# tool-recommender-bot/logparser

Hardware: AMD Instinct MI355X
Metric: GB/s (and lines/s) of 'combined' log parsed per GPU and per 8xMI355X node (higher is better)
Workload: dtype u8

## Files before the change

logparser_amd/csrc/kernels_common.h:

```cpp
#pragma once
#include <hip/hip_runtime.h>

#ifndef LP_KERNEL_TU
#define LP_KERNEL_TU 1
#endif

#include <algorithm>

#include "kernels.h"
#include "lp_device.h"
#include "lp_owner.h"

namespace lp {
namespace {

constexpr int CHUNK = 64 * 1024;
constexpr int NL_THREADS = 256;
constexpr int PW = 64;

typedef uint32_t u32x4 __attribute__((ext_vector_type(4)));

__device__ __forceinline__ uint32_t byte_eq(uint32_t w, uint32_t c4) {
    uint32_t x = w ^ c4;
    return ~(((x & 0x7F7F7F7Fu) + 0x7F7F7F7Fu) | x | 0x7F7F7F7Fu);
}
__device__ __forceinline__ uint32_t bits16(uint32_t m0, uint32_t m1, uint32_t m2, uint32_t m3) {
    return bcls::nib(m0) | (bcls::nib(m1) << 4) | (bcls::nib(m2) << 8) | (bcls::nib(m3) << 12);
}

__device__ __forceinline__ uint32_t term_bits(uint4 v, const uint8_t* p, uint64_t pos, uint64_t nbytes) {
    uint32_t lf = bits16(byte_eq(v.x, 0x0A0A0A0Au), byte_eq(v.y, 0x0A0A0A0Au), byte_eq(v.z, 0x0A0A0A0Au),
                         byte_eq(v.w, 0x0A0A0A0Au));
    uint32_t cr = bits16(byte_eq(v.x, 0x0D0D0D0Du), byte_eq(v.y, 0x0D0D0D0Du), byte_eq(v.z, 0x0D0D0D0Du),
                         byte_eq(v.w, 0x0D0D0D0Du));
    if (pos + 16 > nbytes) {
        const uint32_t live = nbytes > pos ? (1u << (uint32_t)(nbytes - pos)) - 1u : 0u;
        lf &= live;
        cr &= live;
    }
    if (cr) {
        uint32_t next_lf = lf >> 1;
        if ((cr & 0x8000u) && pos + 16 < nbytes && p[pos + 16] == '\n') next_lf |= 0x8000u;
        cr &= ~next_lf;
    }
    return lf | cr;
}
__device__ __forceinline__ uint32_t term16(const uint8_t* p, uint64_t pos, uint64_t nbytes) {
    uint4 v = make_uint4(0, 0, 0, 0);
    if (pos + 16 <= nbytes && ((uintptr_t)(p + pos) & 15) == 0) {
        v = *reinterpret_cast<const uint4*>(p + pos);
    } else {
        uint32_t w[4] = {0, 0, 0, 0};
        for (uint64_t k = pos; k < pos + 16 && k < nbytes; ++k) w[(k - pos) >> 2] |= (uint32_t)p[k] << (8 * ((k - pos) & 3));
        v = make_uint4(w[0], w[1], w[2], w[3]);
    }
    return term_bits(v, p, pos, nbytes);
}

__device__ __forceinline__ int lane_id() {
    return (int)__builtin_amdgcn_mbcnt_hi(~0u, __builtin_amdgcn_mbcnt_lo(~0u, 0u));
}

struct WaveStack {
    uint32_t* base;
    __device__ uint32_t& operator[](int k) const { return base[k * PW]; }
};

template <typename LN>
__device__ __forceinline__ LN owner_line(const LN& L, int own) {
    LN R = L;
    R.o = (uint32_t)__shfl((int)L.o, own);
    R.n = __shfl(L.n, own);
    if constexpr (!LN::has_masks)
        R.b = reinterpret_cast<decltype(L.b)>(__shfl((unsigned long long)(uintptr_t)L.b, own));
    return R;
}

struct WaveLines {
    int64_t li0, li, lend;
    bool active;
    uint64_t s, e, w0, w1;
    int n;
};
__device__ __forceinline__ WaveLines wave_lines(const Columns& C, int64_t wave, int64_t n_lines, uint64_t nbytes) {
    WaveLines W;
    W.li0 = wave * PW;
    W.li = W.li0 + (int64_t)lane_id();
    W.active = W.li < n_lines;
    W.lend = W.li0 + PW < n_lines ? W.li0 + PW : n_lines;
    W.s = W.e = 0;
    if (W.active) {
        W.s = C.line_off[W.li];
        W.e = C.line_off[W.li + 1] - 1;
    }
    W.n = (int)((W.e - W.s) > (uint64_t)0x7FFFFFFF ? 0x7FFFFFFF : (W.e - W.s));
    W.w0 = C.line_off[W.li0] & ~15ull;
    W.w1 = C.line_off[W.lend];
    if (W.w1 > nbytes) W.w1 = nbytes;
    return W;
}

__device__ __forceinline__ int crlf_len(int n, uint32_t last) { return n - (n > 0 && last == '\r' ? 1 : 0); }
__device__ __forceinline__ int crlf_len_hbm(const uint8_t* buf, const WaveLines& W) {
    return W.active ? crlf_len(W.n, W.n > 0 ? buf[W.e - 1] : 0u) : W.n;
}

__device__ __forceinline__ bool stage_window(const uint8_t* __restrict__ buf, uint64_t nbytes, uint64_t w0, uint64_t w1,
                                             uint8_t* win, uint16_t* msk16) {
    const int lane = lane_id();
    const int nv = (int)((w1 - w0 + 15) >> 4);
    const int nv4 = (nv + 3) & ~3;
    uint32_t bad = 0;
    constexpr int SB = 20;
    const uint64_t full_end = nbytes & ~15ull;
    for (int k0 = lane; k0 < nv4; k0 += SB * PW) {
        u32x4 v[SB];
#pragma unroll
        for (int j = 0; j < SB; ++j) {
            const int k = k0 + j * PW;
            const uint64_t p = w0 + 16ull * k;
            v[j] = u32x4{0, 0, 0, 0};
            if (k < nv && p + 16 <= full_end) v[j] = __builtin_nontemporal_load(reinterpret_cast<const u32x4*>(buf + p));
        }
#pragma unroll
        for (int j = 0; j < SB; ++j) {
            const int k = k0 + j * PW;
            if (k >= nv4) continue;
            const uint64_t p = w0 + 16ull * k;
            if (k < nv && p + 16 > full_end) {
                auto word = [&](uint64_t q) {
                    uint32_t w = 0;
#pragma unroll
                    for (int b = 0; b < 4; ++b) w |= q + b < nbytes ? (uint32_t)buf[q + b] << (8 * b) : 0u;
                    return w;
                };
                v[j] = u32x4{word(p), word(p + 4), word(p + 8), word(p + 12)};
            }
            *reinterpret_cast<u32x4*>(win + 16 * k) = v[j];
            uint32_t m0, m1, g = 0, lf, other, cr;
            bcls::classify16p(v[j][0], v[j][1], v[j][2], v[j][3], m0, m1, g, lf, other);
            if (other) bcls::classify16c(v[j][0], v[j][1], v[j][2], v[j][3], g, cr);
            if (k < nv) bad |= g;
            msk16[8 * (k >> 2) + (k & 3)] = (uint16_t)m0;
            msk16[8 * (k >> 2) + 4 + (k & 3)] = (uint16_t)m1;
        }
    }
    return !__any(bad != 0);
}

struct WaveCounts {
    uint32_t act = 0, ok = 0, bad = 0, written = 0;
    uint32_t gathered = 0;
    __device__ __forceinline__ void store(LP_G uint32_t* wave_counts, int64_t wave) const {
        if (lane_id() == 0) {
            uint4 c, d;
            c.x = act;
            c.y = ok;
            c.z = bad;
            c.w = act - ok - bad;
            d.x = written;
            d.y = gathered;
            d.z = d.w = 0;
            uint4* wc = reinterpret_cast<uint4*>(wave_counts + WC_WORDS * (size_t)wave);
            wc[0] = c;
            wc[1] = d;
        }
    }
    __device__ __forceinline__ void store(const Columns& C, int64_t wave) const { store(C.wave_counts, wave); }
};

template <bool MULTI, typename LN>
__device__ __forceinline__ void parse_wave(const Program& P, const Elem* elems, const Columns& C, const LN& L,
                                           bool active, int64_t li, WaveStack stk, bool clean, WaveCounts& WC) {
    LineOut o;
    o.status = ST_OK;
    LP_PROF(1);
    if (active) phase1<MULTI>(P, elems, L, o, stk, C, li, clean, P.n_fmt > 1 ? (int)C.fmt_id[li] : 0);
    LP_PROF(9);
    if (active) write_line(P, o, C, li);
    if (active && !P.has_phase2()) C.arena_base[li] = 0;
    WC.act += (uint32_t)__popcll(__ballot(active));
    WC.ok += (uint32_t)__popcll(__ballot(active && o.status == ST_OK));
    WC.bad += (uint32_t)__popcll(__ballot(active && o.status == ST_BAD));
}

__device__ __forceinline__ u32x4 load16(const uint8_t* __restrict__ buf, uint64_t nbytes, uint64_t p) {
    if (p + 16 <= nbytes) return *reinterpret_cast<const u32x4*>(buf + p);
    uint32_t w[4] = {0, 0, 0, 0};
    for (int c = 0; c < 16; ++c) w[c >> 2] |= p + c < nbytes ? (uint32_t)buf[p + c] << (8 * (c & 3)) : 0u;
    return u32x4{w[0], w[1], w[2], w[3]};
}

__device__ __forceinline__ void load_elems(const Program& P, Elem* s_elems) {
    for (int k = lane_id(); k < P.n_elems; k += PW) s_elems[k] = P.elems[k];
}

__device__ __forceinline__ int lsb64(uint64_t m) { return (int)__builtin_ctzll(m); }
__device__ __forceinline__ int msb64(uint64_t m) { return 63 - (int)__builtin_clzll(m); }

template <typename T>
__device__ __forceinline__ T wave_incl_scan(T x) {
    const int lane = lane_id();
    for (int d = 1; d < 64; d <<= 1) {
        const T y = __shfl_up(x, d);
        if (lane >= d) x += y;
    }
    return x;
}
__device__ __forceinline__ uint32_t wave_incl_scan_dpp(uint32_t x) {
    constexpr int ROW_SHR = 0x110, ROW_BCAST15 = 0x142, ROW_BCAST31 = 0x143;
    x += (uint32_t)__builtin_amdgcn_update_dpp(0, (int)x, ROW_SHR + 1, 0xF, 0xF, false);
    x += (uint32_t)__builtin_amdgcn_update_dpp(0, (int)x, ROW_SHR + 2, 0xF, 0xF, false);
    x += (uint32_t)__builtin_amdgcn_update_dpp(0, (int)x, ROW_SHR + 4, 0xF, 0xF, false);
    x += (uint32_t)__builtin_amdgcn_update_dpp(0, (int)x, ROW_SHR + 8, 0xF, 0xF, false);
    x += (uint32_t)__builtin_amdgcn_update_dpp(0, (int)x, ROW_BCAST15, 0xA, 0xF, false);
    x += (uint32_t)__builtin_amdgcn_update_dpp(0, (int)x, ROW_BCAST31, 0xC, 0xF, false);
    return x;
}
__device__ __forceinline__ uint32_t lane_value(uint32_t x, int l) {
    return (uint32_t)__builtin_amdgcn_readlane((int)x, l);
}
template <typename T>
__device__ __forceinline__ T wave_sum(T x) {
    for (int d = 32; d > 0; d >>= 1) x += __shfl_xor(x, d);
    return x;
}

}
}
```

logparser_amd/csrc/lp_device.h:

```cpp
#pragma once
#include <cstddef>
#include <type_traits>
#include <utility>

#include "lp_program.h"
#include "lp_fixed.h"

namespace lp {

enum : int { ST_OK = 0, ST_BAD = 1, ST_FALLBACK = 2,
             ST_REDO = 3,
             ST_REPAIR = 4 };

#if defined(LP_PROFILE) && defined(__HIP__)
static __device__ unsigned long long g_prof[PROF_WAVES * PROF_POINTS];
#endif
#if defined(LP_PROFILE) && defined(__HIP_DEVICE_COMPILE__)
__device__ __forceinline__ void lp_prof_mark(int k) {
    const unsigned long long t = clock64();
    const unsigned w = blockIdx.x - PROF_W0;
    const uint64_t act = __ballot(1);
    if (w < (unsigned)PROF_WAVES && (int)threadIdx.x % 64 == (int)__builtin_ctzll(act))
        __builtin_nontemporal_store(t, &g_prof[w * PROF_POINTS + k]);
}
__device__ __forceinline__ void lp_prof_acc(int k, unsigned long long& t0) {
    const unsigned long long t = clock64();
    const unsigned w = blockIdx.x - PROF_W0;
    const uint64_t act = __ballot(1);
    if (w < (unsigned)PROF_WAVES && (int)threadIdx.x % 64 == (int)__builtin_ctzll(act))
        g_prof[w * PROF_POINTS + k] += t - t0;
    t0 = t;
}
#define LP_PROF(k) lp_prof_mark(k)
#define LP_PT_DECL unsigned long long lp_pt = clock64();
#define LP_PACC(k) lp_prof_acc(k, lp_pt)
#else
#define LP_PROF(k)
#define LP_PT_DECL
#define LP_PACC(k)
#endif
#if defined(LP_PROFILE) && defined(__HIP_DEVICE_COMPILE__)
#define LP_PROF_EL_BEGIN() unsigned long long lp_el_t = clock64();
#define LP_PROF_EL_END(i) if ((i) < 32) lp_prof_acc(64 + (i), lp_el_t);
#else
#define LP_PROF_EL_BEGIN()
#define LP_PROF_EL_END(i)
#endif

__host__ __device__ LP_INLINE bool is_ws(uint32_t c) { return c == ' ' || (c >= 9 && c <= 13); }
__host__ __device__ LP_INLINE bool is_digit(uint32_t c) { return c - '0' < 10u; }
__host__ __device__ LP_INLINE bool is_hex(uint32_t c) { return is_digit(c) || ((c | 32u) - 'a') < 6u; }
__host__ __device__ LP_INLINE bool is_alpha(uint32_t c) { return ((c | 32u) - 'a') < 26u; }
__host__ __device__ LP_INLINE bool is_alnum(uint32_t c) { return is_alpha(c) || is_digit(c); }
__host__ __device__ LP_INLINE uint32_t hexv(uint32_t c) { return c <= '9' ? c - '0' : (c | 32u) - 'a' + 10; }
__host__ __device__ LP_INLINE int utf8_len(uint32_t c) { return c < 0x80 ? 1 : c < 0xE0 ? 2 : c < 0xF0 ? 3 : 4; }
__host__ __device__ LP_INLINE bool uri_needs_encode(uint32_t c) {
    constexpr uint64_t LO = 0x5000000500000000ull | 0x1FFFFFFFFull;
    constexpr uint64_t HI = 0xB800000178000000ull;
    return c >= 0x80 || (((c < 64 ? LO : HI) >> (c & 63)) & 1u);
}

__host__ __device__ LP_INLINE uint32_t load_word(const uint8_t* p) {
#if defined(__HIP_DEVICE_COMPILE__)
    return *reinterpret_cast<const uint32_t*>(__builtin_assume_aligned(p, 4));
#else
    uint32_t v;
    __builtin_memcpy(&v, p, 4);
    return v;
#endif
}
#if defined(__HIP__)
typedef const __attribute__((address_space(3))) uint8_t* lds_bytes;
typedef const __attribute__((address_space(3))) uint32_t* lds_words;
__device__ LP_INLINE uint32_t load_word(lds_bytes p) { return *(lds_words)p; }
#endif
#if defined(__HIP_DEVICE_COMPILE__) && defined(LP_KERNEL_TU)
__device__ LP_INLINE uint32_t load_word(const LP_G uint8_t* p) {
    return *reinterpret_cast<const LP_G uint32_t*>(__builtin_assume_aligned(p, 4));
}
#endif

enum : int {
    MC_QUOTE = 0,
    MC_UEV = 1,
    MC_WS = 2,
    MC_N = 2
};
__host__ __device__ LP_INLINE uint64_t mask_load(const uint64_t* p) { return *p; }
#if defined(__HIP__)
typedef const __attribute__((address_space(3))) uint64_t* lds_u64;
__device__ LP_INLINE uint64_t mask_load(lds_u64 p) { return *p; }
#endif
struct NoMasks {};
static_assert((int)MC_QUOTE == fs::ACLS_QUOTE, "lp_fixed.h names the QUOTE class by its value");

template <typename Ptr, typename MPtr = NoMasks, int NPL = 2>
struct LineT {
    Ptr b;
    uint32_t o;
    int n;
    MPtr m = MPtr{};
    static constexpr bool has_masks = !std::is_same<MPtr, NoMasks>::value;
    static constexpr bool in_arena = false;
    __host__ __device__ LP_INLINE uint32_t operator[](int i) const { return b[o + i]; }
    __host__ __device__ LP_INLINE uint32_t word(uint32_t w) const { return load_word(b + 4 * w); }
    __host__ __device__ LP_INLINE uint32_t word_or0(uint32_t w) const {
        return 4 * w < o + (uint32_t)n ? load_word(b + 4 * w) : 0u;
    }
    __host__ __device__ LP_INLINE uint64_t mask(int c, uint32_t w) const {
        if constexpr (NPL == 1) {
            return mask_load(m + w);
        } else {
            return mask_load(m + 2 * w + (c == MC_QUOTE ? 0 : 1));
        }
    }
};
using Line = LineT<const uint8_t*>;
using MLine = LineT<const uint8_t*, const uint64_t*>;
using ULine = LineT<const uint8_t*, const uint64_t*, 1>;

template <typename Ptr>
struct ArenaLineT : LineT<Ptr> {
    uint32_t rb;
    static constexpr bool in_arena = true;
};

template <typename LN>
__host__ __device__ LP_INLINE uint64_t src_ref(const LN& L, int x, int n) {
    if constexpr (LN::in_arena) return mkref(L.rb + (uint32_t)x, (uint32_t)n, true);
    else return mkref((uint32_t)x, (uint32_t)n, false);
}

namespace swar {
constexpr uint32_t ONES = 0x01010101u, HI = 0x80808080u, LO7 = 0x7F7F7F7Fu;
__host__ __device__ LP_INLINE uint32_t eq(uint32_t w, uint32_t c) {
    const uint32_t x = w ^ (c * ONES);
    return ~(((x & LO7) + LO7) | x | LO7);
}
__host__ __device__ LP_INLINE uint32_t ge(uint32_t w, uint32_t n) { return (((w & LO7) + (0x80u - n) * ONES) | w) & HI; }
__host__ __device__ LP_INLINE uint32_t lt(uint32_t w, uint32_t n) { return ~ge(w, n) & HI; }
__host__ __device__ LP_INLINE uint32_t ws(uint32_t w) { return eq(w, ' ') | (ge(w, 9) & lt(w, 14)); }
__host__ __device__ LP_INLINE uint32_t digit(uint32_t w) { return ge(w, '0') & lt(w, '9' + 1); }
__host__ __device__ LP_INLINE uint32_t hex(uint32_t w) {
    const uint32_t l = w | 0x20202020u;
    return digit(w) | (ge(l, 'a') & lt(l, 'g') & ~(w & HI));
}
__host__ __device__ LP_INLINE uint32_t upper(uint32_t w) { return ge(w, 'A') & lt(w, 'Z' + 1); }
__host__ __device__ LP_INLINE uint32_t guard_bad(uint32_t w) { return (lt(w, 0x20) & ~eq(w, '\t')) | ge(w, 0x7F); }
__host__ __device__ LP_INLINE uint32_t guard_ctl(uint32_t w) { return (lt(w, 0x20) & ~eq(w, '\t')) | eq(w, 0x7F); }
__host__ __device__ LP_INLINE uint32_t needs_encode(uint32_t w) {
    return lt(w, 0x21) | ge(w, 0x7F) | (ge(w, '{') & lt(w, '~')) | (ge(w, '[') & lt(w, '_')) | eq(w, '`') |
           eq(w, '<') | eq(w, '>') | eq(w, '"');
}
__host__ __device__ LP_INLINE int first(uint32_t m) {
#if defined(__HIP_DEVICE_COMPILE__)
    return (int)(__builtin_ctz(m) >> 3);
#else
    return (int)(__builtin_ctz(m) >> 3);
#endif
}
__host__ __device__ LP_INLINE int last(uint32_t m) { return (int)((31 - __builtin_clz(m)) >> 3); }
__host__ __device__ LP_INLINE int count(uint32_t m) { return __builtin_popcount(m); }
}


namespace bcls {
constexpr uint32_t LO0 = 0x08040081u, LO1 = 0x00080800u;
constexpr uint32_t LO2 = 0x38020200u, LO3 = 0x10502230u;
constexpr uint32_t HI0 = 0x100D0002u, HI1 = 0x20806000u;
__host__ __device__ LP_INLINE uint32_t perm(uint32_t s0, uint32_t s1, uint32_t sel) {
#if defined(__HIP_DEVICE_COMPILE__)
    return __builtin_amdgcn_perm(s0, s1, sel);
#else
    const uint64_t v = ((uint64_t)s0 << 32) | s1;
    uint32_t r = 0;
    for (int i = 0; i < 4; ++i) r |= (uint32_t)((v >> (8 * ((sel >> (8 * i)) & 7))) & 0xFFu) << (8 * i);
    return r;
#endif
}
__host__ __device__ LP_INLINE uint32_t bits(uint32_t w) {
    const uint32_t s = w & 0x07070707u;
    const uint32_t p1 = perm(LO1, LO0, s), p2 = perm(LO3, LO2, s);
    const uint32_t m8 = ((w >> 3) & 0x01010101u) * 0xFFu;
    const uint32_t rl = (p2 & m8) | (p1 & ~m8);
    const uint32_t hb = ((w >> 7) & 0x01010101u) * 0xFFu;
    return (rl & perm(HI1, HI0, (w >> 4) & 0x07070707u) & ~hb) | (hb & 0x08080808u);
}
constexpr uint32_t NA_LO0 = 0x0303010Bu, NA_LO1 = 0x01030301u, NA_LO2 = 0x11010101u, NA_LO3 = 0x47251115u;
constexpr uint32_t NA_HI0 = 0x04020101u, NA_HI1 = 0x50083008u;
__host__ __device__ LP_INLINE uint32_t nonauth_bits(uint32_t w) {
    const uint32_t s = w & 0x07070707u;
    const uint32_t p1 = perm(NA_LO1, NA_LO0, s), p2 = perm(NA_LO3, NA_LO2, s);
    const uint32_t m8 = ((w >> 3) & 0x01010101u) * 0xFFu;
    return ((p2 & m8) | (p1 & ~m8)) & perm(NA_HI1, NA_HI0, (w >> 4) & 0x07070707u);
}
__host__ __device__ LP_INLINE uint32_t nib(uint32_t hb) { return (((hb >> 7) * 0x204081u) >> 21) & 15u; }
__host__ __device__ LP_INLINE uint32_t uev_hb(uint32_t r) { return (((r & swar::LO7) + swar::LO7) | r) & swar::HI; }
__host__ __device__ LP_INLINE uint32_t pack16(uint32_t h0, uint32_t h1, uint32_t h2, uint32_t h3);
__host__ __device__ LP_INLINE uint32_t classify16u(uint32_t w0, uint32_t w1, uint32_t w2, uint32_t w3) {
    return pack16(uev_hb(bits(w0)), uev_hb(bits(w1)), uev_hb(bits(w2)), uev_hb(bits(w3)));
}
__host__ __device__ LP_INLINE uint32_t pack16(uint32_t h0, uint32_t h1, uint32_t h2, uint32_t h3) {
#if defined(__HIP_DEVICE_COMPILE__)
    const uint32_t lo = __builtin_amdgcn_udot4(h1, 0x80402010u, __builtin_amdgcn_udot4(h0, 0x08040201u, 0u, false), false);
    const uint32_t hi = __builtin_amdgcn_udot4(h3, 0x80402010u, __builtin_amdgcn_udot4(h2, 0x08040201u, 0u, false), false);
    return (lo >> 7) | (hi << 1);
#else
    return nib(h0) | (nib(h1) << 4) | (nib(h2) << 8) | (nib(h3) << 12);
#endif
}
__host__ __device__ LP_INLINE void classify16p(uint32_t w0, uint32_t w1, uint32_t w2, uint32_t w3, uint32_t& p0,
                                               uint32_t& p1, uint32_t& bad, uint32_t& lf, uint32_t& other) {
    const uint32_t w[4] = {w0, w1, w2, w3};
    uint32_t q[4], le[4], l[4], o = 0, hi = 0;
    LP_UNROLL for (int k = 0; k < 4; ++k) {
        const uint32_t lo7 = w[k] & swar::LO7;
        le[k] = ~((lo7 + 0x5F5F5F5Fu) | w[k]) & swar::HI;
        const uint32_t lt = ~((lo7 + 0x60606060u) | w[k]) & swar::HI;
        hi |= ((lo7 + 0x01010101u) | w[k]) & swar::HI;
        q[k] = swar::eq(w[k], '"');
        l[k] = swar::eq(w[k], '\n');
        o |= lt & ~l[k];
    }
    p0 = pack16(q[0], q[1], q[2], q[3]);
    p1 = pack16(le[0], le[1], le[2], le[3]);
    lf = pack16(l[0], l[1], l[2], l[3]);
    bad |= hi;
    other = o;
}
__host__ __device__ LP_INLINE void classify16c(uint32_t w0, uint32_t w1, uint32_t w2, uint32_t w3, uint32_t& bad,
                                               uint32_t& cr) {
    const uint32_t w[4] = {w0, w1, w2, w3};
    uint32_t c[4];
    LP_UNROLL for (int k = 0; k < 4; ++k) {
        const uint32_t lt = ~(((w[k] & swar::LO7) + 0x60606060u) | w[k]) & swar::HI;
        c[k] = swar::eq(w[k], '\r');
        bad |= lt & ~(c[k] | swar::eq(w[k], '\n') | swar::eq(w[k], '\t'));
    }
    cr = pack16(c[0], c[1], c[2], c[3]);
}
__host__ __device__ LP_INLINE int class_of(uint32_t c) { return c == '"' ? (int)MC_QUOTE : -1; }
}

inline void build_masks(const uint8_t* buf, uint32_t n, uint64_t* masks) {
    for (uint32_t i = 0; i < MC_N * (n / 64); ++i) masks[i] = 0;
    for (uint32_t k = 0; 16 * k < n; ++k) {
        uint32_t w[4];
        for (int j = 0; j < 4; ++j) __builtin_memcpy(&w[j], buf + 16 * k + 4 * j, 4);
        uint32_t a, b, bad = 0, lf, other;
        bcls::classify16p(w[0], w[1], w[2], w[3], a, b, bad, lf, other);
        const int sh = 16 * (k & 3);
        masks[2 * (k >> 2)] |= (uint64_t)a << sh;
        masks[2 * (k >> 2) + 1] |= (uint64_t)b << sh;
    }
}

inline void build_uev_plane(const uint8_t* buf, uint32_t n, uint64_t* plane) {
    for (uint32_t i = 0; i < n / 64; ++i) plane[i] = 0;
    for (uint32_t k = 0; 16 * k < n; ++k) {
        uint32_t w[4];
        for (int j = 0; j < 4; ++j) __builtin_memcpy(&w[j], buf + 16 * k + 4 * j, 4);
        plane[k >> 2] |= (uint64_t)bcls::classify16u(w[0], w[1], w[2], w[3]) << (16 * (k & 3));
    }
}

__host__ __device__ LP_INLINE int ctz64(uint64_t m) { return __builtin_ctzll(m); }
__host__ __device__ LP_INLINE int msb64(uint64_t m) { return 63 - __builtin_clzll(m); }
__host__ __device__ LP_INLINE int popc64(uint64_t m) { return __builtin_popcountll(m); }

template <typename LN, typename F>
__host__ __device__ LP_INLINE int find_fwd(const LN& L, int from, int to, F cls) {
    if (from >= to) return to;
    const uint32_t A = L.o + (uint32_t)from, E = L.o + (uint32_t)to;
    uint32_t W = A >> 2;
    uint32_t m = cls(L.word(W)) & (swar::HI << (8 * (A & 3)));
    for (;;) {
        if (m) {
            const uint32_t p = (W << 2) + (uint32_t)swar::first(m);
            return p < E ? (int)(p - L.o) : to;
        }
        ++W;
        if ((W << 2) >= E) return to;
        m = cls(L.word(W));
    }
}
template <typename LN, typename F>
__host__ __device__ LP_INLINE int find_bwd(const LN& L, int hi, int lo, F cls) {
    if (hi < lo) return -1;
    const uint32_t A = L.o + (uint32_t)hi, S = L.o + (uint32_t)lo;
    uint32_t W = A >> 2;
    uint32_t m = cls(L.word(W)) & (swar::HI >> (8 * (3 - (A & 3))));
    for (;;) {
        if (m) {
            const uint32_t p = (W << 2) + (uint32_t)swar::last(m);
            return p >= S ? (int)(p - L.o) : -1;
        }
        if ((W << 2) <= S) return -1;
        --W;
        m = cls(L.word(W));
    }
}
template <typename LN, typename F>
__host__ __device__ LP_INLINE uint32_t count_in(const LN& L, int a, int b, F cls) {
    if (a >= b) return 0;
    const uint32_t A = L.o + (uint32_t)a, E = L.o + (uint32_t)b;
    const uint32_t W0 = A >> 2, W1 = (E - 1) >> 2;
    uint32_t c = 0;
    for (uint32_t W = W0; W <= W1; ++W) {
        uint32_t m = cls(L.word(W));
        if (W == W0) m &= swar::HI << (8 * (A & 3));
        if (W == W1) m &= swar::HI >> (8 * (3 - ((E - 1) & 3)));
        c += (uint32_t)swar::count(m);
    }
    return c;
}

template <typename LN>
__host__ __device__ LP_INLINE int mfind_fwd(const LN& L, int c, int from, int to) {
    if (from >= to) return to;
    const uint32_t A = L.o + (uint32_t)from, E = L.o + (uint32_t)to;
    uint32_t W = A >> 6;
    uint64_t m = L.mask(c, W) & (~0ull << (A & 63));
    for (;;) {
        if (m) {
            const uint32_t p = (W << 6) + (uint32_t)ctz64(m);
            return p < E ? (int)(p - L.o) : to;
        }
        ++W;
        if ((W << 6) >= E) return to;
        m = L.mask(c, W);
    }
}
template <typename LN>
__host__ __device__ LP_INLINE int mfind_bwd(const LN& L, int c, int hi, int lo) {
    if (hi < lo) return -1;
    const uint32_t A = L.o + (uint32_t)hi, S = L.o + (uint32_t)lo;
    uint32_t W = A >> 6;
    uint64_t m = L.mask(c, W) & (~0ull >> (63 - (A & 63)));
    for (;;) {
        if (m) {
            const uint32_t p = (W << 6) + (uint32_t)msb64(m);
            return p >= S ? (int)(p - L.o) : -1;
        }
        if ((W << 6) <= S) return -1;
        --W;
        m = L.mask(c, W);
    }
}

template <typename LN, typename F>
__host__ __device__ LP_INLINE bool for_uev(const LN& L, int a, int b, F&& f) {
    if (a >= b) return true;
    const uint32_t A = L.o + (uint32_t)a, E = L.o + (uint32_t)b;
    if constexpr (LN::has_masks) {
        const uint32_t W1 = (E - 1) >> 6;
        const uint64_t last = ~0ull >> (63 - ((E - 1) & 63));
        uint32_t W = A >> 6;
        uint64_t m = L.mask(MC_UEV, W) & (~0ull << (A & 63));
        if (W == W1) m &= last;
        auto next = [&](int& q) {
            while (!m) {
                if (++W > W1) return false;
                m = L.mask(MC_UEV, W);
                if (W == W1) m &= last;
            }
            q = (int)((W << 6) + (uint32_t)ctz64(m) - L.o);
            m &= m - 1;
            return true;
        };
        int q;
        if (!next(q)) return true;
        uint32_t c = L[q];
        for (;;) {
            int q2 = 0;
            const bool more = next(q2);
            const uint32_t c2 = more ? L[q2] : 0u;
            if (!f(q, c)) return false;
            if (!more) return true;
            q = q2;
            c = c2;
        }
    } else {
        const uint32_t W0 = A >> 2, W1 = (E - 1) >> 2;
        for (uint32_t W = W0; W <= W1; ++W) {
            const uint32_t w = L.word(W);
            uint32_t m = bcls::uev_hb(bcls::bits(w));
            if (W == W0) m &= swar::HI << (8 * (A & 3));
            if (W == W1) m &= swar::HI >> (8 * (3 - ((E - 1) & 3)));
            while (m) {
                const int k = swar::first(m);
                m &= m - 1;
                if (!f((int)((W << 2) + (uint32_t)k - L.o), (w >> (8 * k)) & 0xFFu)) return false;
            }
        }
    }
    return true;
}

template <typename LN, typename F>
__host__ __device__ LP_INLINE bool for_uev_w(const LN& L, int a, int b, F&& f) {
    if (a >= b) return true;
    const uint32_t A = L.o + (uint32_t)a, E = L.o + (uint32_t)b;
    if constexpr (LN::has_masks) {
        const uint32_t W1 = (E - 1) >> 6;
        const uint64_t last = ~0ull >> (63 - ((E - 1) & 63));
        uint32_t W = A >> 6;
        uint64_t m = L.mask(MC_UEV, W) & (~0ull << (A & 63));
        if (W == W1) m &= last;
        auto next = [&](int& q) {
            while (!m) {
                if (++W > W1) return false;
                m = L.mask(MC_UEV, W);
                if (W == W1) m &= last;
            }
            q = (int)((W << 6) + (uint32_t)ctz64(m) - L.o);
            m &= m - 1;
            return true;
        };
        int q;
        if (!next(q)) return true;
        uint32_t w = load_u32_at(L, q);
        for (;;) {
            int q2 = 0;
            const bool more = next(q2);
            const uint32_t w2 = more ? load_u32_at(L, q2) : 0u;
            if (!f(q, w)) return false;
            if (!more) return true;
            q = q2;
            w = w2;
        }
    } else {
        return for_uev(L, a, b, [&](int q, uint32_t) { return f(q, load_u32_at(L, q)); });
    }
}

template <typename LN>
__host__ __device__ LP_INLINE uint32_t count_uev(const LN& L, int a, int b) {
    if (a >= b) return 0;
    const uint32_t A = L.o + (uint32_t)a, E = L.o + (uint32_t)b;
    uint32_t c = 0;
    if constexpr (LN::has_masks) {
        const uint32_t W0 = A >> 6, W1 = (E - 1) >> 6;
        for (uint32_t W = W0; W <= W1; ++W) {
            uint64_t m = L.mask(MC_UEV, W);
            if (W == W0) m &= ~0ull << (A & 63);
            if (W == W1) m &= ~0ull >> (63 - ((E - 1) & 63));
            c += (uint32_t)popc64(m);
        }
    } else {
        const uint32_t W0 = A >> 2, W1 = (E - 1) >> 2;
        for (uint32_t W = W0; W <= W1; ++W) {
            uint32_t m = bcls::uev_hb(bcls::bits(L.word(W)));
            if (W == W0) m &= swar::HI << (8 * (A & 3));
            if (W == W1) m &= swar::HI >> (8 * (3 - ((E - 1) & 3)));
            c += (uint32_t)swar::count(m);
        }
    }
    return c;
}

template <typename LN>
__host__ __device__ LP_INLINE int find_ws(const LN& L, int from, int to) {
    if constexpr (LN::has_masks) return mfind_fwd(L, MC_WS, from, to);
    else return find_fwd(L, from, to, [](uint32_t w) { return swar::ws(w); });
}

template <typename LN>
__host__ __device__ LP_INLINE uint32_t load_u32_at(const LN& L, int p) {
    const uint32_t A = L.o + (uint32_t)p;
    const uint32_t w0 = L.word(A >> 2), w1 = L.word_or0((A >> 2) + 1);
#if defined(__HIP_DEVICE_COMPILE__)
    return __builtin_amdgcn_alignbyte(w1, w0, A & 3);
#else
    return (uint32_t)((((uint64_t)w1 << 32) | w0) >> (8 * (A & 3)));
#endif
}

struct Bytes28 {
    uint32_t v[7];
    __host__ __device__ LP_INLINE uint32_t operator[](int k) const { return (v[k >> 2] >> (8 * (k & 3))) & 0xFFu; }
};
template <typename LN>
__host__ __device__ LP_INLINE Bytes28 load28(const LN& L, int p) {
    const uint32_t A = L.o + (uint32_t)p, W = A >> 2, s = A & 3;
    uint32_t w[8];
    LP_UNROLL for (int j = 0; j < 7; ++j) w[j] = L.word(W + j);
    w[7] = L.word_or0(W + 7);
    Bytes28 r;
    LP_UNROLL for (int j = 0; j < 7; ++j) {
#if defined(__HIP_DEVICE_COMPILE__)
        r.v[j] = __builtin_amdgcn_alignbyte(w[j + 1], w[j], s);
#else
        r.v[j] = (uint32_t)((((uint64_t)w[j + 1] << 32) | w[j]) >> (8 * s));
#endif
    }
    return r;
}

template <int N>
struct RegArr {
    static constexpr int size = N;
#if defined(__HIP_DEVICE_COMPILE__)
    typedef uint32_t vec_t __attribute__((ext_vector_type(N)));
    vec_t v;
#else
    uint32_t v[N];
#endif
    template <size_t... J>
    __host__ __device__ LP_INLINE uint32_t get_(int k, std::index_sequence<J...>) const {
        uint32_t r = 0;
        ((r = ((int)J == k) ? v[J] : r), ...);
        return r;
    }
    template <size_t... J>
    __host__ __device__ LP_INLINE void set_(int k, uint32_t x, std::index_sequence<J...>) {
        ((v[J] = ((int)J == k) ? x : v[J]), ...);
    }
    template <typename F, size_t... J>
    __host__ __device__ LP_INLINE void each_(F&& f, std::index_sequence<J...>) const {
        (f((int)J, v[J]), ...);
    }
    __host__ __device__ LP_INLINE uint32_t get(int k) const { return get_(k, std::make_index_sequence<N>{}); }
    __host__ __device__ LP_INLINE uint32_t get_u(int k) const { return v[k]; }
    __host__ __device__ LP_INLINE void set_u(int k, uint32_t x) {
        if ((unsigned)k < (unsigned)N) v[k] = x;
    }
    __host__ __device__ LP_INLINE void set(int k, uint32_t x) { set_(k, x, std::make_index_sequence<N>{}); }
    __host__ __device__ LP_INLINE void fill(uint32_t x) { set_all(x, std::make_index_sequence<N>{}); }
    template <size_t... J>
    __host__ __device__ LP_INLINE void set_all(uint32_t x, std::index_sequence<J...>) { ((v[J] = x), ...); }
    template <typename F>
    __host__ __device__ LP_INLINE void each(F&& f) const { each_(f, std::make_index_sequence<N>{}); }
};

template <typename LN>
__host__ __device__ LP_INLINE bool lit_at(const Program& P, const LN& L, int pos, const ElemV& e) {
    const int len = e.lit_len;
    if (pos + len > L.n) return false;
    if (len <= 4) {
        const uint32_t keep = len == 4 ? 0xFFFFFFFFu : ((1u << (8 * len)) - 1u);
        return ((load_u32_at(L, pos) ^ e.lit4) & keep) == 0;
    }
// ... 3157 lines not shown
```

logparser_amd/csrc/parse_chunk.h:

```cpp
#pragma once
#include "kernels_common.h"

namespace lp {

namespace {


constexpr int MAXS = PW + 1;
#ifndef LP_CHUNK_MAXW
#define LP_CHUNK_MAXW 10
#endif
#ifndef LP_CHUNK_LMAX
#define LP_CHUNK_LMAX 54
#endif
#ifndef LP_MF_WPE
#define LP_MF_WPE 3
#endif
#ifndef LP_CHUNK_LMAX_MF
#define LP_CHUNK_LMAX_MF 58
#endif
constexpr uint64_t CS_AGG = 1ull << 62, CS_INC = 1ull << 63, CS_CNT = CS_AGG - 1;

__device__ __forceinline__ LP_G uint64_t* line_off_w(const Columns& C) { return const_cast<LP_G uint64_t*>(C.line_off); }

constexpr uint64_t CHK_OVF_LINE = 1, CHK_EXCESS = 2, CHK_QUEUE = 3;
__device__ __forceinline__ void check_fail(const Columns& C, uint64_t kind, uint64_t a, uint64_t b, uint64_t c,
                                           uint64_t d) {
    if (atomicAdd(&C.meta->err, 1ull) == 0) {
        C.meta->err_info[0] = kind;
        C.meta->err_info[1] = a;
        C.meta->err_info[2] = b;
        C.meta->err_info[3] = c;
        C.meta->err_info[4] = d;
    }
}

__device__ __forceinline__ void queue_line(const Columns& C, uint64_t li) {
    const uint64_t q = atomicAdd(&C.meta->ovf_lines, 1ull);
    if (q <= (uint64_t)C.cap_lines) C.ovf_lines[q] = (uint32_t)li;
    else check_fail(C, CHK_QUEUE, 0, q, li, (uint64_t)C.cap_lines + 1);
}

__device__ __forceinline__ uint32_t below(uint64_t b) {
    return __builtin_amdgcn_mbcnt_hi((uint32_t)(b >> 32), __builtin_amdgcn_mbcnt_lo((uint32_t)b, 0u));
}

struct ChunkScan {
    uint32_t count;
    uint64_t end_term;
    bool clean;
};

__device__ __forceinline__ ChunkScan stage_chunk(const uint8_t* __restrict__ buf, uint64_t nbytes, uint64_t w0,
                                                 uint64_t w1, uint64_t t_lo, uint64_t t_hi, uint32_t first,
                                                 uint8_t* win, uint16_t* msk16, uint32_t* starts) {
    const int lane = lane_id();
    const int nv = (int)((w1 - w0 + 15) >> 4);
    const int nv4 = (nv + 3) & ~3;
    if ((nv & (PW - 1)) == 0 && w0 + 16ull * nv <= (nbytes & ~15ull)) {
        for (int k0 = 0; k0 < nv; k0 += PW)
            __builtin_amdgcn_global_load_lds((const __attribute__((address_space(1))) void*)(buf + w0 + 16ull * (k0 + lane)),
                                             (__attribute__((address_space(3))) void*)(win + 16 * k0), 16, 0, 0);
        asm volatile("s_waitcnt vmcnt(0)" ::: "memory");
    } else {
        for (int k = lane; k < nv4; k += PW) {
            u32x4 v = u32x4{0, 0, 0, 0};
            if (k < nv) v = load16(buf, nbytes, w0 + 16ull * k);
            *reinterpret_cast<u32x4*>(win + 16 * k) = v;
        }
    }
    const uint32_t nrel = nbytes - w0 < 16ull * (uint64_t)(nv4 + 1) ? (uint32_t)(nbytes - w0) : 16u * (uint32_t)(nv4 + 1);
    const uint32_t tl = (uint32_t)(t_lo - w0), th = (uint32_t)(t_hi - w0);
    uint32_t bad = 0;
    uint32_t run = first;
    uint32_t end_rel = ~0u;
    u32x4 vn = lane < nv4 ? *reinterpret_cast<const u32x4*>(win + 16 * lane) : u32x4{0, 0, 0, 0};
    for (int k0 = 0; k0 < nv4; k0 += PW) {
        const int k = k0 + lane;
        const uint32_t q = 16u * (uint32_t)k;
        const uint32_t r0 = 16u * (uint32_t)k0, r1 = r0 + 16u * PW;
        const bool inner = r0 >= tl && r1 <= th && r1 <= nrel && k0 + PW <= nv;
        uint32_t tm = 0;
        const u32x4 v = vn;
        if (k + PW < nv4) vn = *reinterpret_cast<const u32x4*>(win + 16 * (k + PW));
        if (k < nv4) {
            uint32_t m0, m1, g = 0, lf, other;
            bcls::classify16p(v[0], v[1], v[2], v[3], m0, m1, g, lf, other);
            msk16[8 * (k >> 2) + (k & 3)] = (uint16_t)m0;
            msk16[8 * (k >> 2) + 4 + (k & 3)] = (uint16_t)m1;
            tm = lf;
            if (other) {
                uint32_t cr;
                bcls::classify16c(v[0], v[1], v[2], v[3], g, cr);
                if (cr) {
                    const uint64_t p = w0 + q;
                    uint32_t next_lf = lf >> 1;
                    if ((cr & 0x8000u) && p + 16 < nbytes && buf[p + 16] == '\n') next_lf |= 0x8000u;
                    tm |= cr & ~next_lf;
                }
            }
            if (inner) {
                bad |= g;
            } else {
                if (k < nv) bad |= g;
                if (q + 16 > nrel) tm &= nrel > q ? (1u << (nrel - q)) - 1u : 0u;
            }
        }
        uint32_t ms = tm;
        if (!inner) {
            uint32_t me = 0;
            if (q < tl) ms &= tl - q >= 16 ? 0u : ~0u << (tl - q);
            if (q + 16 > th) {
                const uint32_t lo = th > q ? (1u << (th - q)) - 1u : 0u;
                me = tm & ~lo;
                ms &= lo;
            }
            if (me) end_rel = min(end_rel, q + (uint32_t)__builtin_ctz(me));
        }
        const uint32_t c = (uint32_t)__popc(ms);
        const uint64_t b0 = __ballot(c & 1u), b1 = __ballot(c & 2u);
        uint32_t excl = below(b0) + 2 * below(b1);
        uint32_t tot = (uint32_t)(__popcll(b0) + 2 * __popcll(b1));
        const uint64_t bh = __ballot(c >= 4u);
        if (bh) {
            const uint64_t b2 = __ballot(c & 4u), b3 = __ballot(c & 8u), b4 = __ballot(c & 16u);
            excl += 4 * below(b2) + 8 * below(b3) + 16 * below(b4);
            tot += (uint32_t)(4 * __popcll(b2) + 8 * __popcll(b3) + 16 * __popcll(b4));
        }
        uint32_t r = run + excl;
        run += tot;
        for (uint32_t m = ms; m; m &= m - 1, ++r)
            if (r < (uint32_t)MAXS) starts[r] = q + (uint32_t)__builtin_ctz(m) + 1u;
    }
    ChunkScan S;
    S.count = run;
    for (int d = 32; d > 0; d >>= 1) end_rel = min(end_rel, (uint32_t)__shfl_xor((int)end_rel, d));
    S.end_term = end_rel == ~0u ? ~0ull : w0 + end_rel;
    S.clean = !__any(bad != 0);
    return S;
}

__device__ __forceinline__ void chunk_publish(LP_G uint64_t* st, int64_t c, uint64_t count) {
    if (lane_id() == 0) __hip_atomic_store(&st[c], CS_AGG | count, __ATOMIC_RELAXED, __HIP_MEMORY_SCOPE_AGENT);
}

__device__ __noinline__ void chunk_scanner(LP_G uint64_t* st, int64_t n_chunks) {
    constexpr int PER = 8;
    const int lane = lane_id();
    uint64_t run = 0;
    int64_t c = 0;
    while (c < n_chunks) {
        uint64_t v[PER];
#pragma unroll
        for (int i = 0; i < PER; ++i) {
            const int64_t idx = c + PER * lane + i;
            v[i] = idx < n_chunks ? __hip_atomic_load(&st[idx], __ATOMIC_RELAXED, __HIP_MEMORY_SCOPE_AGENT) : 0ull;
        }
        int pub = 0;
        uint64_t sum = 0;
        bool stop = false;
#pragma unroll
        for (int i = 0; i < PER; ++i) {
            stop = stop || !(v[i] & CS_AGG);
            if (!stop) { sum += v[i] & CS_CNT; ++pub; }
        }
        const uint64_t full = __ballot(pub == PER);
        const int L = full == ~0ull ? PW : (int)__builtin_ctzll(~full);
        const uint64_t mine = lane <= L ? sum : 0ull;
        const uint64_t incl = wave_incl_scan(mine);
        const uint64_t total = __shfl(incl, PW - 1);
        const int pub_L = L < PW ? __shfl(pub, L) : 0;
        if (lane <= L) {
            uint64_t r = run + incl - mine;
#pragma unroll
            for (int i = 0; i < PER; ++i) {
                if (i >= pub) break;
                r += v[i] & CS_CNT;
                __hip_atomic_store(&st[c + PER * lane + i], CS_INC | r, __ATOMIC_RELAXED, __HIP_MEMORY_SCOPE_AGENT);
            }
        }
        const int64_t adv = (int64_t)L * PER + pub_L;
        run += total;
        c += adv;
        if (adv == 0) __builtin_amdgcn_s_sleep(8);
    }
}

constexpr uint32_t CHUNK_WAIT_MAX = 1u << 14;
__device__ __forceinline__ uint64_t chunk_base(LP_G uint64_t* st, int64_t c, uint64_t count, int wait_max) {
    if (wait_max < 0 && (wait_max != -2 || (c & 1))) return ~0ull;
    uint64_t v = 0;
    const uint32_t lim = wait_max <= 0 ? CHUNK_WAIT_MAX : (uint32_t)wait_max;
    if (lane_id() == 0) {
        for (uint32_t it = 0;; ++it) {
            v = __hip_atomic_load(&st[c], __ATOMIC_RELAXED, __HIP_MEMORY_SCOPE_AGENT);
            if (v & CS_INC) break;
            if (it >= lim) { v = ~0ull; break; }
            __builtin_amdgcn_s_sleep(4);
        }
    }
    v = __shfl(v, 0);
    return v == ~0ull ? ~0ull : (v & CS_CNT) - count;
}

__device__ __noinline__ void chunk_excess(const uint8_t* __restrict__ buf, uint64_t nbytes, const Columns& C,
                                         const uint8_t* win, uint64_t w0, uint64_t w1, uint64_t t_lo, uint64_t t_hi,
                                         uint32_t first, uint64_t base, int64_t chunk, uint32_t count) {
    const int lane = lane_id();
    const int nv = (int)((w1 - w0 + 15) >> 4);
    uint32_t run = first;
    for (int k0 = 0; k0 < nv; k0 += PW) {
        const int k = k0 + lane;
        const uint64_t p = w0 + 16ull * k;
        uint32_t ms = 0;
        if (k < nv) {
            const u32x4 v = *reinterpret_cast<const u32x4*>(win + 16 * k);
            ms = term_bits(make_uint4(v[0], v[1], v[2], v[3]), buf, p, nbytes);
            if (p < t_lo) ms &= t_lo - p >= 16 ? 0u : ~0u << (uint32_t)(t_lo - p);
            if (p + 16 > t_hi) ms &= t_hi > p ? (1u << (uint32_t)(t_hi - p)) - 1u : 0u;
        }
        const uint32_t c = (uint32_t)__popc(ms);
        const uint32_t incl = wave_incl_scan(c);
        uint32_t r = run + incl - c;
        run += (uint32_t)__shfl((int)incl, 63);
        for (uint32_t m = ms; m; m &= m - 1, ++r) {
            if (r < (uint32_t)PW) continue;
            const uint64_t li = base + r;
            if ((int64_t)li >= C.cap_lines) continue;
            line_off_w(C)[li] = p + (uint64_t)__builtin_ctz(m) + 1;
            queue_line(C, li);
        }
    }
    if (lane == 0 && run != count) {
        check_fail(C, CHK_EXCESS, (uint64_t)chunk, run, count, base);
        if (C.meta->err_info[1] == (uint64_t)chunk) {
            C.meta->err_info[5] = w0;
            C.meta->err_info[6] = w1;
            C.meta->err_info[7] = t_lo;
            C.meta->err_info[8] = t_hi;
            C.meta->err_info[9] = first;
            C.meta->err_info[10] = (uint64_t)(uintptr_t)win;
            C.meta->err_info[11] = nbytes;
            C.meta->err_info[12] = (uint64_t)(uintptr_t)buf;
        }
    }
}

template <bool LA, bool SIMPLE, bool MF = false, int SHAPE = FS_NONE>
__device__ __forceinline__ void parse_chunk(const uint8_t* __restrict__ buf, uint64_t nbytes, const Program& P,
                                            const Columns& C, const Elem* s_elems, uint8_t* smem, int64_t c,
                                            int64_t n_chunks, uint32_t cb, uint32_t win_cap, uint32_t stk_words,
                                            int direct, int wait_max, bool second) {
    const uint64_t c0 = (uint64_t)c * cb;
    const uint64_t c1 = c0 + cb < nbytes ? c0 + cb : nbytes;
    const int lane = lane_id();
    WaveStack stk{reinterpret_cast<uint32_t*>(smem + 16 * P.n_elems) + lane};
    uint32_t* starts = reinterpret_cast<uint32_t*>(smem + 16 * P.n_elems + 4 * stk_words);
    uint8_t* win = smem + 16 * P.n_elems + 4 * stk_words + 16 * ((4 * MAXS + 15) / 16);
    uint16_t* msk16 = reinterpret_cast<uint16_t*>(win + win_cap);
    const uint64_t w0 = c0 >= 64 ? c0 - 64 : 0;
    const uint64_t w1 = w0 + win_cap < nbytes ? w0 + win_cap : nbytes;
    const uint64_t t_lo = c0 ? c0 - 1 : 0, t_hi = c1 - 1;
    const uint32_t first = c0 == 0 ? 1u : 0u;
    if (first && lane == 0) starts[0] = 0;
    LP_PROF(0);
    const ChunkScan S = stage_chunk(buf, nbytes, w0, w1, t_lo, t_hi, first, win, msk16, starts);
    if (!second) chunk_publish(C.chunk_state, c, S.count);
    LP_PROF(60);
    __syncthreads();
    const uint32_t nl = S.count < (uint32_t)PW ? S.count : (uint32_t)PW;
    const bool has = (uint32_t)lane < nl;
    uint32_t s = 0, e = 0;
    bool known = false;
    if (has) {
        s = starts[lane];
        if ((uint32_t)lane + 1 < S.count) {
            e = starts[lane + 1] - 1;
            known = true;
        } else if (S.end_term != ~0ull) {
            e = (uint32_t)(S.end_term - w0);
            known = true;
        } else if (w1 == nbytes) {
            e = (uint32_t)(nbytes - w0);
            known = true;
        }
    }
    const bool lds_line = has && known && !direct;
    const int n = lds_line ? crlf_len((int)(e - s), e > s ? win[e - 1] : 0u) : 0;
    const LineT<lds_bytes, lds_u64> L{(lds_bytes)win, lds_line ? s : 0u, n, (lds_u64)reinterpret_cast<uint64_t*>(msk16)};
    LineOut o;
    o.status = ST_OK;
    o.tdone = o.smdone = o.bipdone = 0;
    LP_PROF(1);
    uint32_t mword = 0;
    if constexpr (MF) {
        if (lds_line) {
            bool redo = false;
            mword = fmt_match_word<false>(P, s_elems, L, stk, S.clean, &redo, &o.caps);
            const uint32_t mm = mword & 0xFFu;
            if (redo || (mword >> 8) || (mm & (mm - 1))) o.status = ST_REDO;
            else if (mm == 0) o.status = ST_BAD;
            else phase1<true, LA, false, false, true>(P, s_elems, L, o, stk, C, 0, S.clean, __builtin_ctz(mm));
        }
    } else {
#if defined(LP_DFS_IN_CHUNKS)
        if (lds_line) phase1<false, LA, SIMPLE, true>(P, s_elems, L, o, stk, C, 0, S.clean, 0);
#else
        if (lds_line) phase1<false, LA, SIMPLE, false, false, SHAPE>(P, s_elems, L, o, stk, C, 0, S.clean, 0);
#endif
    }
    LP_PROF(9);
    const uint64_t base = chunk_base(C.chunk_state, c, S.count, second ? (int)CHUNK_WAIT_MAX : wait_max);
    if (base == ~0ull) {
        if (lane == 0) {
            const uint64_t q = atomicAdd(&C.meta->deferred, 1ull);
            if (q < (uint64_t)n_chunks) C.deferred_chunks[q] = (uint32_t)c;
            else check_fail(C, CHK_QUEUE, 1, q, (uint64_t)c, (uint64_t)n_chunks);
        }
        return;
    }
    LP_PROF(61);
    const int64_t cap = C.cap_lines;
    const int64_t li = (int64_t)base + lane;
    const bool mine = has && li < cap;
    if (mine) line_off_w(C)[li] = w0 + s;
    if constexpr (MF) {
        if (mine) C.fmt_match[li] = (uint16_t)mword;
    }
    const bool redo = lds_line && o.status == ST_REDO;
    const bool row = mine && lds_line && !redo;
    if (mine && (!lds_line || redo)) queue_line(C, (uint64_t)li);
    {
        const uint32_t nredo = (uint32_t)__popcll(__ballot(mine && redo));
        if (nredo && lane == 0) atomicAdd(&C.meta->dfs_lines, (unsigned long long)nredo);
    }
    if (row) {
        write_line(P, o, C, li);
        if (!P.has_phase2()) C.arena_base[li] = 0;
    }
    if (S.count > (uint32_t)PW)
        chunk_excess(buf, nbytes, C, win, w0, w1, t_lo, t_hi, first, base, c, S.count);
    if (c == n_chunks - 1 && lane == 0) {
        const uint64_t total = base + S.count;
        C.meta->n_lines = total;
        C.meta->cap_ovf = (int64_t)total > cap ? 1ull : 0ull;
        if ((int64_t)total <= cap) {
            const uint8_t last = buf[nbytes - 1];
            line_off_w(C)[total] = last == '\n' || last == '\r' ? nbytes : nbytes + 1;
        }
    }
    WaveCounts WC;
    WC.act = (uint32_t)__popcll(__ballot(row));
    WC.ok = (uint32_t)__popcll(__ballot(row && o.status == ST_OK));
    WC.bad = (uint32_t)__popcll(__ballot(row && o.status == ST_BAD));
    WC.store(C.chunk_counts, c);
    LP_PROF(62);
}

template <bool LA, bool SIMPLE, bool MF, int SHAPE = FS_NONE>
__global__ __launch_bounds__(PW, MF ? LP_MF_WPE : 2) void k_parse_chunks(const uint8_t* __restrict__ buf, uint64_t nbytes,
                                                     const DeviceArgs* __restrict__ args, uint32_t cb, uint32_t win_cap,
                                                     uint32_t stk_words, int direct, int wait_max) {
    const Program& P = args->prog;
    const Columns& C = args->cols;
    const int64_t n_chunks = (int64_t)((nbytes + cb - 1) / cb);
    if (blockIdx.x == 0) {
        chunk_scanner(C.chunk_state, n_chunks);
        return;
    }
    const int64_t c = (int64_t)blockIdx.x - 1;
    if ((uint64_t)c * cb >= nbytes) return;
    extern __shared__ __attribute__((aligned(16))) uint8_t smem[];
    Elem* s_elems = reinterpret_cast<Elem*>(smem);
    load_elems(P, s_elems);
    parse_chunk<LA, SIMPLE, MF, SHAPE>(buf, nbytes, P, C, s_elems, smem, c, n_chunks, cb, win_cap, stk_words, direct,
                                       wait_max, false);
}

template <bool LA, bool SIMPLE, bool MF>
__global__ __launch_bounds__(PW, 2) void k_parse_deferred(const uint8_t* __restrict__ buf, uint64_t nbytes,
                                                       const DeviceArgs* __restrict__ args, uint32_t cb,
                                                       uint32_t win_cap, uint32_t stk_words, int direct) {
    const Program& P = args->prog;
    const Columns& C = args->cols;
    const uint64_t nd = C.meta->deferred;
    if (blockIdx.x >= nd) return;
    const int64_t n_chunks = (int64_t)((nbytes + cb - 1) / cb);
    extern __shared__ __attribute__((aligned(16))) uint8_t smem[];
    Elem* s_elems = reinterpret_cast<Elem*>(smem);
    load_elems(P, s_elems);
    for (uint64_t q = blockIdx.x; q < nd; q += gridDim.x) {
        parse_chunk<LA, SIMPLE, MF>(buf, nbytes, P, C, s_elems, smem, (int64_t)C.deferred_chunks[q], n_chunks, cb,
                                    win_cap, stk_words, direct, 0, true);
        __syncthreads();
    }
}

}
}
```

Baseline: 702.9.

## Classify 64-byte blocks per lane in chunk scan instead of 16-byte vectors

The chunk scan loop now has each lane classify a 64-byte block (four 16-byte vectors) and build 64-bit terminator masks. A wave therefore covers 4KB per iteration, which cuts loop trips and the ballot-based prefix counting per byte by about four times, and the mask writes become single 16-byte stores. In exchange each lane holds more registers, uses more ballot rounds when per-lane counts are high, and the tail handling now works at 64-byte granularity. A profiling marker is also added after the LDS load wait.

Result: faster. 745.0, median of 6 (+6.0%).

```diff
diff --git a/logparser_amd/csrc/kernels_common.h b/logparser_amd/csrc/kernels_common.h
--- a/logparser_amd/csrc/kernels_common.h
+++ b/logparser_amd/csrc/kernels_common.h
@@ -19,6 +19,7 @@
 constexpr int PW = 64;
 
 typedef uint32_t u32x4 __attribute__((ext_vector_type(4)));
+typedef uint64_t u64x2 __attribute__((ext_vector_type(2)));
 
 __device__ __forceinline__ uint32_t byte_eq(uint32_t w, uint32_t c4) {
     uint32_t x = w ^ c4;
diff --git a/logparser_amd/csrc/lp_device.h b/logparser_amd/csrc/lp_device.h
--- a/logparser_amd/csrc/lp_device.h
+++ b/logparser_amd/csrc/lp_device.h
@@ -238,6 +238,24 @@
         bad |= lt & ~(c[k] | swar::eq(w[k], '\n') | swar::eq(w[k], '\t'));
     }
     cr = pack16(c[0], c[1], c[2], c[3]);
+}
+struct Block64 {
+    uint64_t p0, p1, lf;
+    uint32_t g[4];
+    uint32_t other;
+};
+__host__ __device__ LP_INLINE Block64 classify64p(const uint32_t (&w)[16]) {
+    Block64 K;
+    uint32_t a[4], b[4], l[4], o[4];
+    LP_UNROLL for (int j = 0; j < 4; ++j) {
+        K.g[j] = 0;
+        classify16p(w[4 * j], w[4 * j + 1], w[4 * j + 2], w[4 * j + 3], a[j], b[j], K.g[j], l[j], o[j]);
+    }
+    K.p0 = (uint64_t)(a[0] | (a[1] << 16)) | ((uint64_t)(a[2] | (a[3] << 16)) << 32);
+    K.p1 = (uint64_t)(b[0] | (b[1] << 16)) | ((uint64_t)(b[2] | (b[3] << 16)) << 32);
+    K.lf = (uint64_t)(l[0] | (l[1] << 16)) | ((uint64_t)(l[2] | (l[3] << 16)) << 32);
+    K.other = o[0] | o[1] | o[2] | o[3];
+    return K;
 }
 __host__ __device__ LP_INLINE int class_of(uint32_t c) { return c == '"' ? (int)MC_QUOTE : -1; }
 }
diff --git a/logparser_amd/csrc/parse_chunk.h b/logparser_amd/csrc/parse_chunk.h
--- a/logparser_amd/csrc/parse_chunk.h
+++ b/logparser_amd/csrc/parse_chunk.h
@@ -62,6 +62,7 @@
             __builtin_amdgcn_global_load_lds((const __attribute__((address_space(1))) void*)(buf + w0 + 16ull * (k0 + lane)),
                                              (__attribute__((address_space(3))) void*)(win + 16 * k0), 16, 0, 0);
         asm volatile("s_waitcnt vmcnt(0)" ::: "memory");
+        LP_PROF(63);
     } else {
         for (int k = lane; k < nv4; k += PW) {
             u32x4 v = u32x4{0, 0, 0, 0};
@@ -71,66 +72,77 @@
     }
     const uint32_t nrel = nbytes - w0 < 16ull * (uint64_t)(nv4 + 1) ? (uint32_t)(nbytes - w0) : 16u * (uint32_t)(nv4 + 1);
     const uint32_t tl = (uint32_t)(t_lo - w0), th = (uint32_t)(t_hi - w0);
+    const int nb = nv4 >> 2;
     uint32_t bad = 0;
     uint32_t run = first;
     uint32_t end_rel = ~0u;
-    u32x4 vn = lane < nv4 ? *reinterpret_cast<const u32x4*>(win + 16 * lane) : u32x4{0, 0, 0, 0};
-    for (int k0 = 0; k0 < nv4; k0 += PW) {
-        const int k = k0 + lane;
-        const uint32_t q = 16u * (uint32_t)k;
-        const uint32_t r0 = 16u * (uint32_t)k0, r1 = r0 + 16u * PW;
-        const bool inner = r0 >= tl && r1 <= th && r1 <= nrel && k0 + PW <= nv;
-        uint32_t tm = 0;
-        const u32x4 v = vn;
-        if (k + PW < nv4) vn = *reinterpret_cast<const u32x4*>(win + 16 * (k + PW));
-        if (k < nv4) {
-            uint32_t m0, m1, g = 0, lf, other;
-            bcls::classify16p(v[0], v[1], v[2], v[3], m0, m1, g, lf, other);
-            msk16[8 * (k >> 2) + (k & 3)] = (uint16_t)m0;
-            msk16[8 * (k >> 2) + 4 + (k & 3)] = (uint16_t)m1;
-            tm = lf;
-            if (other) {
-                uint32_t cr;
-                bcls::classify16c(v[0], v[1], v[2], v[3], g, cr);
+    u32x4 vn[4];
+    LP_UNROLL for (int j = 0; j < 4; ++j)
+        vn[j] = lane < nb ? *reinterpret_cast<const u32x4*>(win + 64 * lane + 16 * j) : u32x4{0, 0, 0, 0};
+    for (int b0 = 0; b0 < nb; b0 += PW) {
+        const int B = b0 + lane;
+        const uint32_t q = 64u * (uint32_t)B;
+        const uint32_t r0 = 64u * (uint32_t)b0, r1 = r0 + 64u * PW;
+        const bool inner = r0 >= tl && r1 <= th && r1 <= nrel && 4 * (b0 + PW) <= nv;
+        uint64_t tm = 0;
+        uint32_t w[16];
+        LP_UNROLL for (int j = 0; j < 16; ++j) w[j] = vn[j >> 2][j & 3];
+        if (B + PW < nb) {
+            LP_UNROLL for (int j = 0; j < 4; ++j) vn[j] = *reinterpret_cast<const u32x4*>(win + 64 * (B + PW) + 16 * j);
+        }
+        if (B < nb) {
+            bcls::Block64 K = bcls::classify64p(w);
+            *reinterpret_cast<u64x2*>(msk16 + 8 * B) = u64x2{K.p0, K.p1};
+            tm = K.lf;
+            if (K.other) {
+                uint64_t cr = 0;
+                LP_UNROLL for (int j = 0; j < 4; ++j) {
+                    uint32_t c;
+                    bcls::classify16c(w[4 * j], w[4 * j + 1], w[4 * j + 2], w[4 * j + 3], K.g[j], c);
+                    cr |= (uint64_t)c << (16 * j);
+                }
                 if (cr) {
                     const uint64_t p = w0 + q;
-                    uint32_t next_lf = lf >> 1;
-                    if ((cr & 0x8000u) && p + 16 < nbytes && buf[p + 16] == '\n') next_lf |= 0x8000u;
+                    uint64_t next_lf = K.lf >> 1;
+                    if ((cr >> 63) && p + 64 < nbytes && buf[p + 64] == '\n') next_lf |= 1ull << 63;
                     tm |= cr & ~next_lf;
                 }
             }
             if (inner) {
-                bad |= g;
+                bad |= K.g[0] | K.g[1] | K.g[2] | K.g[3];
             } else {
-                if (k < nv) bad |= g;
-                if (q + 16 > nrel) tm &= nrel > q ? (1u << (nrel - q)) - 1u : 0u;
+                LP_UNROLL for (int j = 0; j < 4; ++j)
+                    if (4 * B + j < nv) bad |= K.g[j];
+                if (q + 64 > nrel) tm &= nrel > q ? (1ull << (nrel - q)) - 1ull : 0ull;
             }
         }
-        uint32_t ms = tm;
+        uint64_t ms = tm;
         if (!inner) {
-            uint32_t me = 0;
-            if (q < tl) ms &= tl - q >= 16 ? 0u : ~0u << (tl - q);
-            if (q + 16 > th) {
-                const uint32_t lo = th > q ? (1u << (th - q)) - 1u : 0u;
+            uint64_t me = 0;
+            if (q < tl) ms &= tl - q >= 64 ? 0ull : ~0ull << (tl - q);
+            if (q + 64 > th) {
+                const uint64_t lo = th > q ? (1ull << (th - q)) - 1ull : 0ull;
                 me = tm & ~lo;
                 ms &= lo;
             }
-            if (me) end_rel = min(end_rel, q + (uint32_t)__builtin_ctz(me));
-        }
-        const uint32_t c = (uint32_t)__popc(ms);
-        const uint64_t b0 = __ballot(c & 1u), b1 = __ballot(c & 2u);
-        uint32_t excl = below(b0) + 2 * below(b1);
-        uint32_t tot = (uint32_t)(__popcll(b0) + 2 * __popcll(b1));
+            if (me) end_rel = min(end_rel, q + (uint32_t)__builtin_ctzll(me));
+        }
+        const uint32_t c = (uint32_t)__popcll(ms);
+        const uint64_t b0m = __ballot(c & 1u), b1m = __ballot(c & 2u);
+        uint32_t excl = below(b0m) + 2 * below(b1m);
+        uint32_t tot = (uint32_t)(__popcll(b0m) + 2 * __popcll(b1m));
         const uint64_t bh = __ballot(c >= 4u);
         if (bh) {
-            const uint64_t b2 = __ballot(c & 4u), b3 = __ballot(c & 8u), b4 = __ballot(c & 16u);
-            excl += 4 * below(b2) + 8 * below(b3) + 16 * below(b4);
-            tot += (uint32_t)(4 * __popcll(b2) + 8 * __popcll(b3) + 16 * __popcll(b4));
+            LP_UNROLL for (int k = 2; k < 7; ++k) {
+                const uint64_t bk = __ballot(c & (1u << k));
+                excl += below(bk) << k;
+                tot += (uint32_t)__popcll(bk) << k;
+            }
         }
         uint32_t r = run + excl;
         run += tot;
-        for (uint32_t m = ms; m; m &= m - 1, ++r)
-            if (r < (uint32_t)MAXS) starts[r] = q + (uint32_t)__builtin_ctz(m) + 1u;
+        for (uint64_t m = ms; m; m &= m - 1, ++r)
+            if (r < (uint32_t)MAXS) starts[r] = q + (uint32_t)__builtin_ctzll(m) + 1u;
     }
     ChunkScan S;
     S.count = run;
```
